# xiaoxubeii/kubernetes-schedule-simulator

Hardware: AMD Instinct MI355X
Metric: pods scheduled/sec + node-evals/sec at 100k nodes, 1/2/4/8 MI355X (higher is better)
Workload: dtype int64; 1 GPU; C3: 100000 nodes, 1000000-pod queue, default predicates + LeastRequested(1) + BalancedResourceAllocation(1); nodes=100000, global_batch=35715, mode=persistent, blocks=256, parallelism=single-gpu

## Files before the change

### kubernetes-schedule-simulator_amd/csrc/ksim_pfast.hip

```cpp
#include <algorithm>

#include "ksim_decide.h"
#include "ksim_f64.h"
#include "ksim_fast.h"
#include "ksim_phist.h"
#include "ksim_tree.h"
#include "ksim_wave.h"
#include "ksim_xchg.h"

using namespace kf64;

namespace {

#ifndef KSIM_PF_BS
#define KSIM_PF_BS 512
#endif
constexpr int BS = KSIM_PF_BS;
constexpr int NW = BS / 64;
constexpr int RW = NW - 1;
constexpr int RT = RW * 64;
constexpr int MAXB = 4;
constexpr int MAXG = 64 * MAXB;
constexpr int NSLOT = 4;
constexpr int FIXSTRIDE = 16;
constexpr int RING = 16;
constexpr int RING_FILL = 8;
constexpr uint64_t SPIN_LIMIT_TICKS = 200000000ull;
constexpr int ANSLOT = 8;

using ksimx::gu64;
__device__ __forceinline__ uint64_t* spec_at(uint64_t* gr, int slot, int b) {
  return gr + slot * MAXG + (b % MAXB) * 64 + b / MAXB;
}
__device__ __forceinline__ uint64_t* fix_at(uint64_t* gr, int slot) { return gr + NSLOT * MAXG + slot * FIXSTRIDE; }
#ifndef KSIM_NREP
#define KSIM_NREP 8
#endif
constexpr int NREP = KSIM_NREP;

constexpr int REP_STRIDE = 2112;
static_assert(NSLOT * MAXG + NSLOT * FIXSTRIDE <= REP_STRIDE, "replica overlap");

constexpr double EXACT_LIM = 281474976710656.0;
__device__ __forceinline__ uint32_t gtag(uint64_t v) { return (uint32_t)(v >> 56); }
__device__ __forceinline__ bool gstop(uint64_t v) { return (v >> 55) & 1; }
__device__ __forceinline__ int32_t gfit(uint64_t v) { return (int32_t)((v >> 42) & 0x1FFF); }
__device__ __forceinline__ int32_t gcnt(uint64_t v) { return (int32_t)((v >> 29) & 0x1FFF); }
__device__ __forceinline__ int32_t gscore(uint64_t v) { return ((int32_t)((uint32_t)v << 3)) >> 3; }
__device__ __forceinline__ uint64_t gpack(uint64_t tag, int32_t f, int32_t n, int32_t m) {
  return (tag << 56) | ((uint64_t)(uint32_t)f << 42) | ((uint64_t)(uint32_t)n << 29) | ((uint64_t)(uint32_t)m & 0x1FFFFFFFull);
}

__device__ __forceinline__ void lds_barrier() {
  __builtin_amdgcn_fence(__ATOMIC_RELEASE, "workgroup", "local");
  __builtin_amdgcn_s_barrier();
  __builtin_amdgcn_fence(__ATOMIC_ACQUIRE, "workgroup", "local");
}

#ifdef KSIM_PROBE
#define PROBE(k) do { if (KSIM_PROBE == (k)) __builtin_amdgcn_s_sleep(8); } while (0)
#else
#define PROBE(k) do { } while (0)
#endif

#ifdef KSIM_STAMPS
#define STAMP(k)                                       \
  do {                                                 \
    const uint64_t t_ = __builtin_amdgcn_s_memtime(); \
    st_acc[k] += t_ - t_prev;                         \
    t_prev = t_;                                      \
  } while (0)
#define OSTAMP(k)                                                          \
  do {                                                                     \
    const uint64_t t_ = __builtin_amdgcn_s_memtime();                     \
    if (lane == 0) atomicAdd((unsigned long long*)&a.dbg[k], t_ - o_prev); \
    o_prev = t_;                                                           \
  } while (0)
#else
#define STAMP(k) \
  do {           \
  } while (0)
#define OSTAMP(k) \
  do {            \
  } while (0)
#endif

}

struct PfArgs {
  int64_t n, chunk, first, end;
  const int64_t* alloc_cpu;
  const int64_t* alloc_mem;
  const int32_t* allowed_pods;
  const uint32_t* flags;
  int64_t* req_cpu;
  int64_t* req_mem;
  int64_t* nz_cpu;
  int64_t* nz_mem;
  int32_t* pod_count;
  const ksim_pod* pods;
  uint64_t* counter;
  int64_t* cursor;
  int32_t* out_node;
  int32_t* out_reasons;
  int32_t* err;
  uint64_t* dbg;
  uint64_t* granules;
  uint32_t preds;
  int32_t no_prio, collect;
  int32_t wl, wm, wb;
  int32_t rank, world;
  int64_t node_base;
  uint32_t xtag_base;
  uint64_t* xchg;
  uint64_t* peers[KSIM_MAX_RANKS];
  uint64_t start_ticks;
  double* mirror;
  const int32_t* tcls;
  const KsimTreeClass* tclass;
  int32_t ncls;
};

namespace {

struct FRows {
  double *ac, *am, *rc, *rm, *zc, *zm, *yc, *ym;
  int32_t *allowed, *count;
  uint32_t* fl;
  int32_t* ev;
  int32_t* ev2;
  uint32_t* rm2;
  uint32_t* rma;
  int16_t* cache;
  uint16_t* hist;
};

constexpr int LDS_ROW_BYTES = 8 * 8 + 8 * 4;
constexpr int LDS_ROW_BYTES_STREAM = 7 * 4;

extern __shared__ __attribute__((aligned(16))) char kf_smem[];

template <bool STREAM>
__device__ __forceinline__ FRows carve(int rows, const PfArgs& a, int64_t lo) {
  FRows r;
  if (STREAM) {
    double* m = a.mirror + lo;
    const int64_t n = a.n;
    r.ac = m; r.am = m + n; r.rc = m + 2 * n; r.rm = m + 3 * n;
    r.zc = m + 4 * n; r.zm = m + 5 * n; r.yc = nullptr; r.ym = nullptr;
    r.allowed = const_cast<int32_t*>(a.allowed_pods) + lo;
    r.count = a.pod_count + lo;
    r.fl = const_cast<uint32_t*>(a.flags) + lo;
    int32_t* q = reinterpret_cast<int32_t*>(kf_smem);
    r.ev = q;
    r.ev2 = q + 2 * rows;
    r.rm2 = reinterpret_cast<uint32_t*>(q + 3 * rows);
    r.rma = r.rm2 + 2 * rows;
    r.cache = nullptr;
    r.hist = nullptr;
    return r;
  }
  double* d = reinterpret_cast<double*>(kf_smem);
  r.ac = d; r.am = d + rows; r.rc = d + 2 * rows; r.rm = d + 3 * rows;
  r.zc = d + 4 * rows; r.zm = d + 5 * rows; r.yc = d + 6 * rows; r.ym = d + 7 * rows;
  int32_t* q = reinterpret_cast<int32_t*>(d + 8 * rows);
  r.allowed = q; r.count = q + rows;
  r.fl = reinterpret_cast<uint32_t*>(q + 2 * rows);
  r.ev = q + 3 * rows;
  r.ev2 = q + 5 * rows;
  r.rm2 = reinterpret_cast<uint32_t*>(q + 6 * rows);
  r.cache = reinterpret_cast<int16_t*>(q + 8 * rows);
  r.hist = reinterpret_cast<uint16_t*>(reinterpret_cast<char*>(r.cache) + (((size_t)a.ncls * rows * 2 + 15) & ~(size_t)15));
  return r;
}

typedef __attribute__((address_space(1))) const uint64_t cgu64;
typedef __attribute__((address_space(1))) const int32_t cgi32;
__device__ __forceinline__ double ld_l2(const double* p) {
  return __builtin_bit_cast(double, __hip_atomic_load((cgu64*)p, __ATOMIC_RELAXED, __HIP_MEMORY_SCOPE_AGENT));
}
__device__ __forceinline__ int32_t ld_l2(const int32_t* p) {
  return __hip_atomic_load((cgi32*)p, __ATOMIC_RELAXED, __HIP_MEMORY_SCOPE_AGENT);
}
__device__ __forceinline__ FRow load_frow_l2(const FRows& R, int32_t j) {
  FRow r;
  r.ac = ld_l2(R.ac + j); r.am = ld_l2(R.am + j); r.rc = ld_l2(R.rc + j); r.rm = ld_l2(R.rm + j);
  r.zc = ld_l2(R.zc + j); r.zm = ld_l2(R.zm + j);
  r.yc = r.ac != 0.0 ? 1.0 / r.ac : 0.0;
  r.ym = r.am != 0.0 ? 1.0 / r.am : 0.0;
  r.allowed = ld_l2(R.allowed + j); r.count = ld_l2(R.count + j);
  r.fl = (uint32_t)ld_l2(reinterpret_cast<const int32_t*>(R.fl) + j);
  return r;
}

template <bool STREAM>
__device__ __forceinline__ FRow load_frow(const FRows& R, int32_t j) {
  FRow r;
  r.ac = R.ac[j]; r.am = R.am[j]; r.rc = R.rc[j]; r.rm = R.rm[j]; r.zc = R.zc[j]; r.zm = R.zm[j];
  if (STREAM) {
    r.yc = r.ac != 0.0 ? 1.0 / r.ac : 0.0;
    r.ym = r.am != 0.0 ? 1.0 / r.am : 0.0;
  } else {
    r.yc = R.yc[j]; r.ym = R.ym[j];
  }
  r.allowed = R.allowed[j]; r.count = R.count[j]; r.fl = R.fl[j];
  return r;
}

struct Top2 {
  int32_t f, m1, c1, m2, c2;
};

}

template <int NPT, bool STREAM, bool CACHE, bool HIST = false>
__global__ __launch_bounds__(BS) void ksim_pfast_kernel(PfArgs a) {
  static_assert(!(STREAM && CACHE), "the cached form keeps the rows in LDS");
  static_assert(!HIST || CACHE, "the histograms count the cached evaluations");
  __shared__ int32_t s_wst[HIST ? 1 : 2][HIST ? 1 : RW][5];
  __shared__ uint64_t s_bm[2][NPT][RW];
  __shared__ int32_t s_wg[2][5];
  __shared__ int32_t s_fix[2][2];
  __shared__ int32_t s_hist[KSIM_NREASONS];
  __shared__ int32_t s_mode[2], s_own[2];
  __shared__ int32_t s_arr;
  __shared__ int32_t s_prow[2];
  __shared__ double s_pdel[2][4];
  __shared__ double s_pval[4];
  __shared__ int32_t s_pcnt;
  __shared__ __attribute__((aligned(16))) ksim_pod s_pod[RING];
  __shared__ int32_t s_pcls[CACHE ? RING : 1];
  __shared__ KsimTreeClass s_tcl[CACHE ? KSIM_TREE_MAX_CLASSES : 1];
#ifdef KSIM_STAMPS
  uint64_t st_acc[16] = {};
#endif

  const int tid = threadIdx.x, lane = tid & 63, wv = tid >> 6;
  const int rt = tid - 64;
  const int G = gridDim.x;
  const int me = blockIdx.x;
  const int64_t chunk = a.chunk;
  const int64_t lo = (int64_t)me * chunk;
  const int64_t hi = (lo + chunk < a.n) ? lo + chunk : a.n;
  const int32_t nrows = (int32_t)(hi - lo);
  const FRows R = carve<STREAM>((int)chunk, a, lo);
  const uint32_t preds = a.preds;
  const bool no_prio = a.no_prio != 0;
  const EvCfg EC = make_evcfg(preds, no_prio, a.wl, a.wm, a.wb);
  int32_t* const top_list = reinterpret_cast<int32_t*>(R.rm2 + chunk);
  uint64_t* const granules = a.granules;
  constexpr int NR = STREAM ? 1 : NREP;
  uint64_t* const my_rep = NR == 1 ? granules : granules + (me % NR) * REP_STRIDE;

  for (int32_t j = tid; j < (STREAM ? 0 : nrows); j += BS) {
    const int64_t i = lo + j;
    const double ac = (double)a.alloc_cpu[i], am = (double)a.alloc_mem[i];
    R.ac[j] = ac; R.am[j] = am;
    R.yc[j] = ac != 0.0 ? 1.0 / ac : 0.0;
    R.ym[j] = am != 0.0 ? 1.0 / am : 0.0;
    R.rc[j] = (double)a.req_cpu[i]; R.rm[j] = (double)a.req_mem[i];
    R.zc[j] = (double)a.nz_cpu[i]; R.zm[j] = (double)a.nz_mem[i];
    R.allowed[j] = a.allowed_pods[i]; R.count[j] = a.pod_count[i]; R.fl[j] = a.flags[i];
  }
  auto ring_load = [&](int64_t p0, uint4& v, int32_t& cl) {
    const int64_t p = p0 + lane / 8;
    if (p < a.end) v = reinterpret_cast<const uint4*>(&a.pods[p])[lane % 8];
    if (CACHE && lane < RING_FILL && p0 + lane < a.end) cl = a.tcls[p0 + lane];
  };
  auto ring_store = [&](int64_t p0, const uint4& v, int32_t cl) {
    const int64_t p = p0 + lane / 8;
    if (p < a.end) reinterpret_cast<uint4*>(&s_pod[p % RING])[lane % 8] = v;
    if (CACHE && lane < RING_FILL && p0 + lane < a.end) s_pcls[(p0 + lane) % RING] = cl;
  };
  uint4 ring_next = make_uint4(0, 0, 0, 0);
  int32_t ring_next_cl = 0;
  if (wv == 1) {
    uint4 v;
    int32_t cl = 0;
    ring_load(a.first, v, cl);
    ring_load(a.first + RING_FILL, ring_next, ring_next_cl);
    ring_store(a.first, v, cl);
  }
  if (CACHE)
    for (int k = tid; k < a.ncls; k += BS) s_tcl[k] = a.tclass[k];
  if (tid == 0) { s_fix[a.first & 1][0] = -1; s_arr = 0; s_prow[0] = s_prow[1] = -1; }
  uint64_t counter = *a.counter;
  __syncthreads();
  auto cls_fpod = [&](int k) -> FPod {
    const KsimTreeClass& t = s_tcl[k];
    return FPod{t.rq_c, t.rq_m, t.nz_c, t.nz_m, 0.0, 0.0, t.anyreq, t.be};
  };
  if (CACHE) {
    const int tot = a.ncls * nrows;
    uint32_t* const hw = reinterpret_cast<uint32_t*>(R.hist);
    if (HIST) {
      for (int i = tid; i < a.ncls * (KSIM_PHIST_BUCKETS / 2); i += BS) hw[i] = 0;
      __syncthreads();
    }
    for (int idx = tid; idx < tot; idx += BS) {
      const int k = idx / nrows, j = idx - k * nrows;
      uint32_t rm;
      const int32_t ev = feval(EC, cls_fpod(k), load_frow<false>(R, j), rm);
      R.cache[k * chunk + j] = (int16_t)ev;
      if (HIST && ev >= 0) atomicAdd(&hw[k * (KSIM_PHIST_BUCKETS / 2) + khist::word(ev)], khist::unit(ev));
    }
    __syncthreads();
  }

  auto ptag = [&](int64_t p) -> uint64_t { return (uint64_t)((p - a.first + 1) & 0xFF); };
  auto wave_stats = [&](const int32_t (&e)[NPT], int buf, int w) {
    int32_t v = -1, nf = 0;
#pragma unroll
    for (int k = 0; k < NPT; ++k) {
      nf += __popcll(__ballot(e[k] >= 0));
      v = e[k] > v ? e[k] : v;
    }
    const int32_t m1 = ksimw::max_i32(v);
    int32_t v2 = -1;
#pragma unroll
    for (int k = 0; k < NPT; ++k) v2 = (e[k] < m1 && e[k] > v2) ? e[k] : v2;
    const int32_t m2 = ksimw::max_i32(v2);
    int32_t c1 = 0, c2 = 0;
#pragma unroll
    for (int k = 0; k < NPT; ++k) {
      const uint64_t bm = m1 < 0 ? 0ull : __ballot(e[k] == m1);
      c1 += __popcll(bm);
      c2 += m2 < 0 ? 0 : __popcll(__ballot(e[k] == m2));
      if (lane == 0) s_bm[buf][k][w - 1] = bm;
    }
    if (lane == 0) {
      s_wst[buf][w - 1][0] = nf; s_wst[buf][w - 1][1] = m1; s_wst[buf][w - 1][2] = c1;
      s_wst[buf][w - 1][3] = m2; s_wst[buf][w - 1][4] = c2;
    }
  };
  auto arrive_publish = [&](int64_t p, int buf) {
    __builtin_amdgcn_fence(__ATOMIC_RELEASE, "workgroup", "local");
    int32_t old = 0;
    if (lane == 0) old = atomicAdd(&s_arr, 1);
    old = __builtin_amdgcn_readfirstlane(old);
    if ((old + 1) % RW == 0) {
      __builtin_amdgcn_fence(__ATOMIC_ACQUIRE, "workgroup", "local");
      const bool in = lane < RW;
      const int w = in ? lane : 0;
      const int32_t f = in ? s_wst[buf][w][0] : 0;
      const int32_t a1 = s_wst[buf][w][1], n1 = in ? s_wst[buf][w][2] : 0;
      const int32_t a2 = s_wst[buf][w][3], n2 = in ? s_wst[buf][w][4] : 0;
      Top2 t;
      t.f = ksimw::sum_i32(f);
      t.m1 = ksimw::max_i32(n1 ? a1 : -1);
      t.c1 = ksimw::sum_i32((n1 && a1 == t.m1) ? n1 : 0);
      t.m2 = ksimw::max_i32(n1 && a1 < t.m1 ? a1 : (n2 ? a2 : -1));
      t.c2 = ksimw::sum_i32(((n1 && a1 == t.m2) ? n1 : 0) + ((n2 && a2 == t.m2) ? n2 : 0));
      if (t.m2 < 0) t.c2 = 0;
      if (lane == 0) {
        s_wg[buf][0] = t.f; s_wg[buf][1] = t.m1; s_wg[buf][2] = t.c1; s_wg[buf][3] = t.m2; s_wg[buf][4] = t.c2;
        if (NR == 1) ksimx::store_agent((gu64*)spec_at(granules, (int)(p % NSLOT), me), gpack(ptag(p), t.f, t.c1, t.m1));
      }
      if (NR > 1 && lane < NR)
        ksimx::store_agent((gu64*)spec_at(granules + lane * REP_STRIDE, (int)(p % NSLOT), me), gpack(ptag(p), t.f, t.c1, t.m1));
    }
  };
  auto hist_publish = [&](int64_t p, int buf) {
    const int cls = s_pcls[p % RING];
    const int32_t h = R.hist[cls * KSIM_PHIST_BUCKETS + lane];
    const int32_t M = khist::top(__ballot(h != 0));
    if (wv == 1) {
      const int32_t F = ksimw::sum_i32(h);
      const int32_t C = __builtin_amdgcn_readlane(h, M < 0 ? 0 : M);
      if (lane == 0) {
        s_wg[buf][0] = F; s_wg[buf][1] = M; s_wg[buf][2] = C;
        if (NR == 1) ksimx::store_agent((gu64*)spec_at(granules, (int)(p % NSLOT), me), gpack(ptag(p), F, C, M));
      }
      if (NR > 1 && lane < NR)
        ksimx::store_agent((gu64*)spec_at(granules + lane * REP_STRIDE, (int)(p % NSLOT), me), gpack(ptag(p), F, C, M));
    }
    const int16_t* c1 = R.cache + cls * chunk;
#pragma unroll
    for (int k = 0; k < NPT; ++k) {
      const int32_t j = k * RT + rt;
      const uint64_t bm = __ballot(M >= 0 && j < nrows && (int32_t)c1[j] == M);
      if (lane == 0) s_bm[buf][k][wv - 1] = bm;
    }
  };
  struct Segs {
    uint64_t m;
    int32_t cnt, base, total;
  };
  auto seg_prepare = [&](int buf) -> Segs {
    constexpr int S = NPT * RW;
    const int32_t M = s_wg[buf][1];
    Segs sg;
    sg.m = 0;
    if (lane < S) {
      const int k = NPT - 1 - lane / RW, w = RW - 1 - lane % RW;
      if constexpr (HIST) sg.m = M >= 0 ? s_bm[buf][k][w] : 0ull;
      else sg.m = (M >= 0 && s_wst[buf][w][1] == M) ? s_bm[buf][k][w] : 0ull;
    }
    sg.cnt = __popcll(sg.m);
    const int32_t incl = ksimw::prefix_incl_i32(sg.cnt);
    sg.base = incl - sg.cnt;
    sg.total = __builtin_amdgcn_readlane(incl, 63);
    return sg;
  };
  auto seg_select = [&](const Segs& sg, int32_t rank) -> int32_t {
    const uint64_t hs = __ballot(sg.cnt != 0 && rank >= sg.base && rank < sg.base + sg.cnt);
    if (rank >= sg.total || !hs) return -1;
    const int t = __builtin_ctzll(hs);
    const uint64_t ms = ((uint64_t)(uint32_t)__builtin_amdgcn_readlane((int32_t)(sg.m >> 32), t) << 32) |
                        (uint64_t)(uint32_t)__builtin_amdgcn_readlane((int32_t)sg.m, t);
    const int32_t r = rank - __builtin_amdgcn_readlane(sg.base, t);
    const uint64_t hb = __ballot(((ms >> lane) & 1ull) && __popcll(ms >> lane) - 1 == r);
    if (!hb) return -1;
    const int k = NPT - 1 - t / RW, w = RW - 1 - t % RW;
    return k * RT + w * 64 + __builtin_ctzll(hb);
  };

  auto build_top_list = [&](int buf) {
    constexpr int S = NPT * RW;
    const int32_t M = s_wg[buf][1];
    uint64_t m = 0;
    if (lane < S) {
      const int k = NPT - 1 - lane / RW, w = RW - 1 - lane % RW;
      m = (M >= 0 && s_wst[buf][w][1] == M) ? s_bm[buf][k][w] : 0ull;
    }
    const int32_t cnt = __popcll(m);
    const int32_t base = ksimw::prefix_incl_i32(cnt) - cnt;
    uint64_t live = __ballot(cnt != 0);
    while (live) {
      const int t = __builtin_ctzll(live);
      live &= live - 1;
      const uint64_t ms = ((uint64_t)(uint32_t)__builtin_amdgcn_readlane((int32_t)(m >> 32), t) << 32) |
                          (uint64_t)(uint32_t)__builtin_amdgcn_readlane((int32_t)m, t);
      const int32_t b0 = __builtin_amdgcn_readlane(base, t);
      const int k = NPT - 1 - t / RW, w = RW - 1 - t % RW;
      if ((ms >> lane) & 1ull) top_list[b0 + __popcll(ms >> lane) - 1] = k * RT + w * 64 + lane;
    }
  };

  uint32_t A_rm[STREAM ? 1 : NPT], B_rm[STREAM ? 1 : NPT];
  if (wv > 0) {
    const FPod P0 = load_fpod(s_pod[a.first % RING]);
    int32_t e[NPT];
    int32_t* ev = R.ev + (a.first & 1) * chunk;
#pragma unroll
    for (int k = 0; k < NPT; ++k) {
      const int32_t j = k * RT + rt;
      e[k] = -1;
      uint32_t& am = A_rm[STREAM ? 0 : k];
      am = 0;
      if (CACHE) {
        if (j < nrows) e[k] = R.cache[s_pcls[a.first % RING] * chunk + j];
      } else if (j < nrows) {
        e[k] = feval(EC, P0, load_frow<STREAM>(R, j), am);
        if (STREAM) R.rma[(a.first & 1) * chunk + j] = am;
        ev[j] = e[k];
      }
    }
    if constexpr (HIST) {
      hist_publish(a.first, (int)(a.first & 1));
    } else {
      wave_stats(e, (int)(a.first & 1), wv);
      arrive_publish(a.first, (int)(a.first & 1));
    }
  }
  int X = -1;
  int64_t stop_at = a.end;
  lds_barrier();
#ifdef KSIM_STAMPS
  uint64_t t_prev = __builtin_amdgcn_s_memtime();
  uint64_t tb_prev = t_prev, bw_busy = 0, bw_wait = 0;
#endif

  int64_t last = a.first;
  for (int64_t pod = a.first; pod < a.end; ++pod) {
    last = pod;
    const bool has_next = pod + 1 < a.end;
    const int pb = (int)(pod & 1);
    const int nb = (int)((pod + 1) & 1);
    int32_t jsel = -1;
    uint64_t stopbit = 0;
    FRow jrow;
    int32_t e_new = -1;
    uint32_t m_new = 0;
    int32_t hM_old = -1, hM_new = -1;
    int32_t hcls = 0, hrow = 0, hF0 = 0;
    int32_t he_old = -1;
    double hdel[4] = {0.0, 0.0, 0.0, 0.0};
#ifdef KSIM_STAMPS
    uint64_t o_prev = 0;
#endif

    if (wv == 0) {
      Segs sg{};
      if (STREAM) build_top_list(pb);
      else sg = seg_prepare(pb);
      if constexpr (HIST) {
        if (has_next) {
          hcls = s_pcls[(pod + 1) % RING];
          hrow = R.hist[hcls * KSIM_PHIST_BUCKETS + lane];
          hF0 = ksimw::sum_i32(hrow);
          hM_old = khist::top(__ballot(hrow != 0));
        }
        const ksim_pod& Pp = s_pod[pod % RING];
        hdel[0] = (double)Pp.add_cpu; hdel[1] = (double)Pp.add_mem; hdel[2] = (double)Pp.nz_cpu; hdel[3] = (double)Pp.nz_mem;
      }
      STAMP(1);
      const uint64_t tag = ptag(pod);
      const int slot = (int)(pod % NSLOT);
      uint64_t g[MAXB], fx = 0;
      bool ok = false;
      const uint64_t t0 = __builtin_amdgcn_s_memrealtime();
      for (;;) {
#pragma unroll
        for (int j = 0; j < MAXB; ++j) g[j] = ksimx::load_agent((gu64*)my_rep + slot * MAXG + j * 64 + lane);
        fx = ksimx::load_agent((gu64*)fix_at(my_rep, slot));
        bool mine = X < 0 || gtag(fx) == tag;
#pragma unroll
        for (int j = 0; j < MAXB; ++j) {
          const int b = lane * MAXB + j;
          mine &= (b >= G) || b == X || gtag(g[j]) == tag;
        }
        if (__all(mine)) {
          ok = true;
#pragma unroll
          for (int j = 0; j < MAXB; ++j) g[j] = (lane * MAXB + j == X) ? fx : g[j];
          break;
        }
        if (__builtin_amdgcn_s_memrealtime() - t0 > SPIN_LIMIT_TICKS) break;
        __builtin_amdgcn_s_sleep(1);
      }
      STAMP(2);
      PROBE(3);
      int32_t f = 0, lm = -1;
#pragma unroll
      for (int j = 0; j < MAXB; ++j) {
        g[j] = (lane * MAXB + j < G) ? g[j] : 0;
        f += gfit(g[j]);
        lm = (gcnt(g[j]) && gscore(g[j]) > lm) ? gscore(g[j]) : lm;
      }
      const int32_t Fl = ksimw::sum_i32(f);
      const int32_t Ml = ksimw::max_i32(lm);
      int32_t bm[MAXB], tot = 0;
#pragma unroll
      for (int j = 0; j < MAXB; ++j) {
        bm[j] = (gcnt(g[j]) && gscore(g[j]) == Ml) ? gcnt(g[j]) : 0;
        tot += bm[j];
      }
      const int32_t pre = ksimw::prefix_incl_i32(tot);
      const int32_t Cl = __builtin_amdgcn_readlane(pre, 63);
      int32_t F = Fl, M0 = Ml;
      uint32_t C = (uint32_t)Cl;
      int64_t above_r = 0;
      bool stop_any = ok && X >= 0 && gstop(fx);
      if (a.world > 1 && ok) {
        const uint64_t at = (uint64_t)(uint32_t)(a.xtag_base + (uint32_t)(pod - a.first) + 1u) << 32;
        const int aslot = (int)(pod % ANSLOT);
        if (me == 0 && lane < a.world) {
          uint64_t* dst = a.peers[lane] + ((int64_t)aslot * KSIM_MAX_RANKS + a.rank) * 4;
          ksimx::store_system(dst, at | (uint32_t)Fl);
          ksimx::store_system(dst + 1, at | (stop_any ? 0x80000000ull : 0ull) | (uint32_t)Cl);
          ksimx::store_system(dst + 2, at | (uint32_t)Ml);
        }
        const bool rl = lane < a.world;
        const uint64_t* src = a.xchg + ((int64_t)aslot * KSIM_MAX_RANKS + (rl ? lane : 0)) * 4;
        uint64_t w0 = 0, w1 = 0, w2 = 0;
        const uint64_t hi = 0xFFFFFFFF00000000ull;
        for (;;) {
          w0 = ksimx::load_system(src);
          w1 = ksimx::load_system(src + 1);
          w2 = ksimx::load_system(src + 2);
          if (__all(!rl || ((w0 & hi) == at && (w1 & hi) == at && (w2 & hi) == at))) break;
          const uint64_t lim = (pod == a.first) ? a.start_ticks : SPIN_LIMIT_TICKS;
          if (__builtin_amdgcn_s_memrealtime() - t0 > lim) { ok = false; break; }
          __builtin_amdgcn_s_sleep(1);
        }
        const int32_t Fr = rl ? (int32_t)(uint32_t)w0 : 0, Cr = rl ? (int32_t)((uint32_t)w1 & 0x7FFFFFFFu) : 0;
        const int32_t Mr = (rl && Cr) ? (int32_t)(uint32_t)w2 : -1;
        F = ksimw::sum_i32(Fr);
        M0 = ksimw::max_i32(Mr);
        const int32_t Cm = (Cr && Mr == M0) ? Cr : 0;
        const int32_t pr = ksimw::prefix_incl_i32(Cm);
        C = (uint32_t)__builtin_amdgcn_readlane(pr, 63);
        above_r = (int64_t)C - __builtin_amdgcn_readlane(pr, a.rank);
        stop_any = __any(rl && ((w1 >> 31) & 1));
      }
      const uint32_t Cs = C ? C : 1u;
      const int64_t ix = ksim_select_ix(counter, Cs);
      const int64_t ixl = ix - above_r;
      const int64_t above = (int64_t)Cl - pre;
      const bool hit = Ml == M0 && tot > 0 && ixl >= above && ixl < above + tot;
      int32_t found = -1;
      int64_t rr = ixl - above;
#pragma unroll
      for (int j = MAXB - 1; j >= 0; --j) {
        const bool here = found < 0 && rr < bm[j];
        found = here ? lane * MAXB + j : found;
        rr = (found < 0) ? rr - bm[j] : rr;
      }
      const uint64_t hb = __ballot(hit);
      const int src = __builtin_ffsll((long long)hb) - 1;
      const int blk = hb ? __builtin_amdgcn_readlane(found, src) : -1;
      const int rank = hb ? __builtin_amdgcn_readlane((int32_t)rr, src) : 0;
      int mode;
      if (!ok) mode = -1;
      else if (stop_any) mode = -2;
      else if (F == 0) mode = 0;
      else if (hb) mode = blk >= 0 ? 2 : -1;
      else mode = a.world > 1 ? 3 : -1;
      if (mode >= 2 && F > 1) counter += 1;
      if (lane == 0 && mode == -1) atomicOr(a.err, ok ? 2 : 4);
      STAMP(3);
#ifdef KSIM_STAMPS
      o_prev = __builtin_amdgcn_s_memtime();
#endif
      if (mode == 2 && blk == me) {
        jsel = STREAM ? (rank < s_wg[pb][2] ? top_list[rank] : -1) : seg_select(sg, rank);
        if (jsel < 0 || jsel >= nrows) {
          jsel = -1;
          mode = -1;
          if (lane == 0) atomicOr(a.err, 2);
        } else if (HIST) {
          const double s0 = R.rc[jsel] + hdel[0], s1 = R.rm[jsel] + hdel[1], s2 = R.zc[jsel] + hdel[2], s3 = R.zm[jsel] + hdel[3];
          if (has_next) he_old = (int32_t)R.cache[hcls * chunk + jsel];
          stopbit = ((s0 >= EXACT_LIM) | (s1 >= EXACT_LIM) | (s2 >= EXACT_LIM) | (s3 >= EXACT_LIM)) ? (1ull << 55) : 0ull;
        } else if (!STREAM) {
          const ksim_pod& Pp = s_pod[pod % RING];
          stopbit = (R.rc[jsel] + (double)Pp.add_cpu >= EXACT_LIM || R.rm[jsel] + (double)Pp.add_mem >= EXACT_LIM ||
                     R.zc[jsel] + (double)Pp.nz_cpu >= EXACT_LIM || R.zm[jsel] + (double)Pp.nz_mem >= EXACT_LIM)
                        ? (1ull << 55)
                        : 0ull;
        } else if (has_next) {
          jrow = load_frow_l2(R, jsel);
          if (jsel != s_prow[nb]) {
            const FRow r2 = plus(jrow, load_fpod(s_pod[pod % RING]));
            e_new = feval(EC, load_fpod(s_pod[(pod + 1) % RING]), r2, m_new);
            stopbit = (r2.rc >= EXACT_LIM || r2.rm >= EXACT_LIM || r2.zc >= EXACT_LIM || r2.zm >= EXACT_LIM) ? (1ull << 55) : 0ull;
          }
        }
        OSTAMP(22);
      }
      if ((mode == 0 || mode == 3) && me == 0 && lane == 0) a.out_node[pod] = mode == 0 ? -1 : -2;
      if (lane == 0) {
        s_mode[pb] = mode;
        s_own[pb] = jsel;
        if (STREAM) {
          s_prow[pb] = jsel;
          if (jsel >= 0) {
            const ksim_pod& Pp = s_pod[pod % RING];
            s_pdel[pb][0] = (double)Pp.add_cpu; s_pdel[pb][1] = (double)Pp.add_mem;
            s_pdel[pb][2] = (double)Pp.nz_cpu; s_pdel[pb][3] = (double)Pp.nz_mem;
          }
        }
      }
      X = mode == 2 ? blk : -1;
      STAMP(6);
    } else {
      const int32_t prow = STREAM ? s_prow[nb] : -1;
      auto apply_commit = [&](FRow& r, int32_t j) {
        r.rc += s_pdel[nb][0]; r.rm += s_pdel[nb][1]; r.zc += s_pdel[nb][2]; r.zm += s_pdel[nb][3]; r.count += 1;
        R.rc[j] = r.rc; R.rm[j] = r.rm; R.zc[j] = r.zc; R.zm[j] = r.zm; R.count[j] = r.count;
        s_pval[0] = r.rc; s_pval[1] = r.rm; s_pval[2] = r.zc; s_pval[3] = r.zm; s_pcnt = r.count;
      };
      if (STREAM && !has_next && prow >= 0) {
#pragma unroll
        for (int k = 0; k < NPT; ++k) {
          const int32_t j = k * RT + rt;
          if (j == prow) {
            FRow r = load_frow<STREAM>(R, j);
            apply_commit(r, j);
          }
        }
      }
      if (has_next) {
      const bool refill = wv == 1 && ((pod - a.first) % RING_FILL) == 0;
      if (refill) ring_store(pod + RING_FILL, ring_next, ring_next_cl);
      uint4 rv;
      int32_t rcl = 0;
      if (refill) ring_load(pod + 2 * RING_FILL, rv, rcl);
#ifdef KSIM_STAMPS
      const uint64_t te0 = __builtin_amdgcn_s_memtime();
#endif
      PROBE(4);
      const FPod P = load_fpod(s_pod[pod % RING]);
      const FPod Q = load_fpod(s_pod[(pod + 1) % RING]);
#ifdef KSIM_STAMPS
      uint64_t tw = __builtin_amdgcn_s_memtime();
      if (tid == 64) st_acc[8] += tw - te0;
#define WSTAMP(k) do { const uint64_t t_ = __builtin_amdgcn_s_memtime(); if (tid == 64) st_acc[k] += t_ - tw; tw = t_; } while (0)
#else
#define WSTAMP(k) do { } while (0)
#endif
      int32_t e[NPT];
      FRow rk[STREAM ? 1 : NPT];
      int32_t* evn = R.ev + nb * chunk;
      if (CACHE) {
        if constexpr (HIST) {
          WSTAMP(9);
          hist_publish(pod + 1, nb);
          WSTAMP(10);
        } else {
          const int16_t* c1 = R.cache + s_pcls[(pod + 1) % RING] * chunk;
#pragma unroll
          for (int k = 0; k < NPT; ++k) {
            const int32_t j = k * RT + rt;
            e[k] = j < nrows ? (int32_t)c1[j] : -1;
          }
          WSTAMP(9);
          wave_stats(e, nb, wv);
          WSTAMP(10);
          arrive_publish(pod + 1, nb);
        }
        const int32_t M0 = s_wg[pb][1];
        const int16_t* c0 = R.cache + s_pcls[pod % RING] * chunk;
#pragma unroll
        for (int k = 0; k < NPT; ++k) {
          const int32_t j = k * RT + rt;
          if (M0 >= 0 && j < nrows && (int32_t)c0[j] == M0) {
            uint32_t m2;
            R.ev2[j] = feval(EC, Q, plus(load_frow<false>(R, j), P), m2);
            R.rm2[j] = m2;
          }
        }
      } else {
#pragma unroll
      for (int k = 0; k < NPT; ++k) {
        const int32_t j = k * RT + rt;
        e[k] = -1;
        uint32_t& bm = B_rm[STREAM ? 0 : k];
        bm = 0;
        if (j < nrows) {
          FRow r = load_frow<STREAM>(R, j);
          if (STREAM && j == prow) apply_commit(r, j);
          e[k] = feval(EC, Q, r, bm);
          evn[j] = e[k];
          if (STREAM) {
            R.rma[nb * chunk + j] = bm;
          } else {
            rk[STREAM ? 0 : k] = r;
          }
        }
      }
      WSTAMP(9);
      wave_stats(e, nb, wv);
      WSTAMP(10);
      PROBE(1);
      arrive_publish(pod + 1, nb);
      if (!STREAM) {
#pragma unroll
        for (int k = 0; k < NPT; ++k) {
          const int32_t j = k * RT + rt;
          if (j < nrows) {
            uint32_t m2;
            R.ev2[j] = feval(EC, Q, plus(rk[STREAM ? 0 : k], P), m2);
            R.rm2[j] = m2;
          }
        }
      }
      }
      WSTAMP(11);
#ifdef KSIM_STAMPS
      if (tid == 64) st_acc[5] += __builtin_amdgcn_s_memtime() - te0;
#endif
      if (refill) { ring_next = rv; ring_next_cl = rcl; }
      }
      if (STREAM && prow >= 0 && wv == 1 + (prow % RT) / 64) asm volatile("s_waitcnt vmcnt(0)" ::: "memory");
    }
#ifdef KSIM_STAMPS
    const uint64_t tb0 = __builtin_amdgcn_s_memtime();
#endif
    lds_barrier();
#ifdef KSIM_STAMPS
    {
      const uint64_t tb1 = __builtin_amdgcn_s_memtime();
      bw_busy += tb0 - tb_prev;
      bw_wait += tb1 - tb0;
      tb_prev = tb1;
    }
#endif
    STAMP(7);
    const int mode = s_mode[pb];
    if (mode < 0) {
      if (mode == -2) stop_at = pod;
      break;
    }
    const int32_t own = s_own[pb];

    if (own >= 0) {
      if (wv == 0) {
        OSTAMP(17);
        if (has_next) {
          if (STREAM && jsel == s_prow[nb]) {
            FRow r = jrow;
            r.rc = s_pval[0]; r.rm = s_pval[1]; r.zc = s_pval[2]; r.zm = s_pval[3]; r.count = s_pcnt;
            const FRow r2 = plus(r, load_fpod(s_pod[pod % RING]));
            e_new = feval(EC, load_fpod(s_pod[(pod + 1) % RING]), r2, m_new);
            stopbit = (r2.rc >= EXACT_LIM || r2.rm >= EXACT_LIM || r2.zc >= EXACT_LIM || r2.zm >= EXACT_LIM) ? (1ull << 55) : 0ull;
          }
          if (!STREAM) { e_new = R.ev2[jsel]; m_new = R.rm2[jsel]; }
          int32_t e_old, f0, m1 = -1, c1 = 0, m2 = -1, c2 = 0;
          if constexpr (HIST) {
            e_old = he_old;
            f0 = hF0;
          } else {
            e_old = CACHE ? (int32_t)R.cache[s_pcls[(pod + 1) % RING] * chunk + jsel] : R.ev[nb * chunk + jsel];
            f0 = s_wg[nb][0]; m1 = s_wg[nb][1]; c1 = s_wg[nb][2]; m2 = s_wg[nb][3]; c2 = s_wg[nb][4];
          }
          const bool rem = e_old >= 0, add = e_new >= 0;
          const int32_t Ff = f0 - (rem ? 1 : 0) + (add ? 1 : 0);
          int32_t M, Cn;
          if constexpr (HIST) {
            const int32_t h = khist::adjusted(hrow, lane, e_old, e_new);
            M = khist::top(__ballot(h != 0));
            Cn = __builtin_amdgcn_readlane(h, M < 0 ? 0 : M);
            hM_new = M;
          } else {
            const int32_t c1a = c1 - ((rem && e_old == m1) ? 1 : 0);
            const int32_t mb = c1a ? m1 : (c2 ? m2 : -1), cb = c1a ? c1a : c2;
            const bool up = add && (cb == 0 || e_new > mb), eq = add && !up && e_new == mb;
            M = up ? e_new : mb;
            Cn = up ? 1 : cb + (eq ? 1 : 0);
          }
          PROBE(2);
          if (NR > 1 && lane < NR)
            ksimx::store_agent((gu64*)fix_at(granules + lane * REP_STRIDE, (int)((pod + 1) % NSLOT)),
                          gpack(ptag(pod + 1), Ff, Cn, Cn ? M : -1) | stopbit);
          if (lane == 0) {
            if (NR == 1)
              ksimx::store_agent((gu64*)fix_at(granules, (int)((pod + 1) % NSLOT)), gpack(ptag(pod + 1), Ff, Cn, Cn ? M : -1) | stopbit);
            s_wg[nb][0] = Ff; s_wg[nb][1] = Cn ? M : -1; s_wg[nb][2] = Cn;
          }
        }
        OSTAMP(18);
        if (CACHE) {
          const FRow r2 = plus(load_frow<false>(R, jsel), load_fpod(s_pod[pod % RING]));
          if (lane < a.ncls) {
            uint32_t rm;
            const int32_t en = feval(EC, cls_fpod(lane), r2, rm);
            if constexpr (HIST) khist::move(R.hist + lane * KSIM_PHIST_BUCKETS, (int32_t)R.cache[lane * chunk + jsel], en);
            R.cache[lane * chunk + jsel] = (int16_t)en;
          }
        }
        if (lane == 0) {
          if (!STREAM) {
            const ksim_pod& Pp = s_pod[pod % RING];
            R.rc[jsel] += (double)Pp.add_cpu; R.rm[jsel] += (double)Pp.add_mem;
            R.zc[jsel] += (double)Pp.nz_cpu; R.zm[jsel] += (double)Pp.nz_mem;
            R.count[jsel] += 1;
          }
          if (stopbit) atomicOr(a.err, 8);
          a.out_node[pod] = (int32_t)(a.node_base + lo + jsel);
          if (has_next) {
            R.ev[nb * chunk + jsel] = e_new;
            s_fix[nb][0] = jsel;
            s_fix[nb][1] = (int32_t)m_new;
          } else {
            s_fix[nb][0] = -1;
          }
        }
      }
      lds_barrier();
      if (HIST && wv == 0 && has_next) {
        if (hM_new == hM_old) {
          if (lane == 0 && hM_new >= 0) {
            uint64_t& m = s_bm[nb][jsel / RT][(jsel % RT) / 64];
            const uint64_t bit = 1ull << (jsel & 63);
            m = e_new == hM_new ? (m | bit) : (m & ~bit);
          }
        } else {
          const int16_t* c1 = R.cache + s_pcls[(pod + 1) % RING] * chunk;
          for (int sgi = 0; sgi < NPT * RW; ++sgi) {
            const int32_t j = sgi * 64 + lane;
            const uint64_t bm = __ballot(hM_new >= 0 && j < nrows && (int32_t)c1[j] == hM_new);
            if (lane == 0) s_bm[nb][sgi / RW][sgi % RW] = bm;
          }
        }
        OSTAMP(19);
#ifdef KSIM_STAMPS
        if (lane == 0) atomicAdd((unsigned long long*)&a.dbg[21], 1ull);
#endif
      }
      if (!HIST && wv == 0 && has_next) {
        const int w = 1 + (jsel % RT) / 64;
        int32_t e[NPT];
#pragma unroll
        for (int k = 0; k < NPT; ++k) {
          const int32_t j = k * RT + (w - 1) * 64 + lane;
          e[k] = j < nrows ? (CACHE ? (int32_t)R.cache[s_pcls[(pod + 1) % RING] * chunk + j] : R.ev[nb * chunk + j]) : -1;
        }
        wave_stats(e, nb, w);
        OSTAMP(19);
#ifdef KSIM_STAMPS
        if (lane == 0) atomicAdd((unsigned long long*)&a.dbg[21], 1ull);
#endif
      }
    } else if (wv == 0 && lane == 0) {
      s_fix[nb][0] = -1;
    }

    if (mode == 0 && a.collect && a.out_reasons) {
      if (tid < KSIM_NREASONS) s_hist[tid] = 0;
      lds_barrier();
      if (wv > 0) {
        const int32_t fr = s_fix[pb][0];
        const uint32_t fmk = (uint32_t)s_fix[pb][1];
#pragma unroll
        for (int k = 0; k < NPT; ++k) {
          const int32_t j = k * RT + rt;
          uint32_t rm = (j == fr) ? fmk : !STREAM ? A_rm[STREAM ? 0 : k] : (j < nrows ? R.rma[pb * chunk + j] : 0u);
          if (CACHE) {
            rm = 0;
            if (j < nrows) (void)feval(EC, load_fpod(s_pod[pod % RING]), load_frow<false>(R, j), rm);
          }
          for (int r = 0; r < KSIM_NREASONS; ++r) {
            const int32_t n = __popcll(__ballot((rm >> r) & 1u));
            if (lane == 0 && n) atomicAdd(&s_hist[r], n);
          }
        }
      }
      lds_barrier();
      if (tid < KSIM_NREASONS && s_hist[tid]) atomicAdd(&a.out_reasons[pod * KSIM_NREASONS + tid], s_hist[tid]);
    }
    STAMP(4);
    if (wv > 0) {
#pragma unroll
      for (int k = 0; k < (STREAM ? 0 : NPT); ++k) A_rm[k] = B_rm[k];
    }
  }

  __syncthreads();
  if (STREAM) {
    if (tid == 0) {
      const int32_t pr = s_prow[last & 1];
      if (pr >= 0) {
        const double* d = s_pdel[last & 1];
        R.rc[pr] += d[0]; R.rm[pr] += d[1]; R.zc[pr] += d[2]; R.zm[pr] += d[3]; R.count[pr] += 1;
        if (R.rc[pr] >= EXACT_LIM || R.rm[pr] >= EXACT_LIM || R.zc[pr] >= EXACT_LIM || R.zm[pr] >= EXACT_LIM)
          atomicOr(a.err, 8);
      }
    }
    __syncthreads();
  }
  for (int32_t j = tid; j < nrows; j += BS) {
    const int64_t i = lo + j;
    a.req_cpu[i] = (int64_t)R.rc[j]; a.req_mem[i] = (int64_t)R.rm[j];
    a.nz_cpu[i] = (int64_t)R.zc[j]; a.nz_mem[i] = (int64_t)R.zm[j];
    a.pod_count[i] = R.count[j];
  }
  if (me == 0 && tid == 0) {
    *a.counter = counter;
    *a.cursor = stop_at;
  }
#ifdef KSIM_STAMPS
  if (me == 0 && lane == 0) {
    atomicAdd((unsigned long long*)&a.dbg[32 + wv], bw_busy);
    atomicAdd((unsigned long long*)&a.dbg[40 + wv], bw_wait);
  }
  if (me == 0 && tid == 0)
    for (int k = 0; k < 16; ++k) a.dbg[k] += (k == 5 || (k >= 8 && k <= 11)) ? 0 : st_acc[k];
  if (me == 0 && tid == 64)
    for (int k : {5, 8, 9, 10, 11}) a.dbg[k] += st_acc[k];
#endif
}

static constexpr int PF_LDS_BUDGET = 150 * 1024;

extern "C" int ksim_pfast_config(int64_t n, int max_grid, int stream, int* grid, int* lds_rows) {
  int dev = 0;
  hipDeviceProp_t p;
  if (hipGetDevice(&dev) != hipSuccess || hipGetDeviceProperties(&p, dev) != hipSuccess) return 0;
  int g = p.multiProcessorCount;
  if (max_grid > 0 && g > max_grid) g = max_grid;
  if (g <= 0 || n <= 0) return 0;
  if (g > MAXG) g = MAXG;
  if (n < (int64_t)g * 64) g = (int)((n + 63) / 64);
  if (g < 1) g = 1;
  const int64_t chunk = (n + g - 1) / g;
  if (stream) {
    if (chunk * LDS_ROW_BYTES_STREAM > PF_LDS_BUDGET || chunk > 9 * RT) return 0;
  } else if (chunk * LDS_ROW_BYTES > PF_LDS_BUDGET || chunk > 4 * RT) {
    return 0;
  }
  *grid = g;
  *lds_rows = (int)chunk;
  return 1;
}

extern "C" size_t ksim_pfast_granule_bytes(void) { return (size_t)NREP * REP_STRIDE * sizeof(uint64_t); }

extern "C" size_t ksim_shard_lx_offset(void) { return (size_t)ANSLOT * KSIM_MAX_RANKS * 4; }
extern "C" size_t ksim_shard_xchg_bytes(void) {
  return (ksim_shard_lx_offset() + (size_t)KSIM_LX_SLOTS * KSIM_MAX_RANKS * (KSIM_LX_REC + KSIM_PX_REC)) *
         sizeof(uint64_t);
}

__global__ __launch_bounds__(256) void ksim_pstream_prepare_kernel(const int64_t* __restrict__ ac, const int64_t* __restrict__ am,
                                                                    const int64_t* __restrict__ rc, const int64_t* __restrict__ rm,
                                                                    const int64_t* __restrict__ zc, const int64_t* __restrict__ zm,
                                                                    int64_t n, double* __restrict__ m) {
  for (int64_t i = (int64_t)blockIdx.x * blockDim.x + threadIdx.x; i < n; i += (int64_t)gridDim.x * blockDim.x) {
    const double dac = (double)ac[i], dam = (double)am[i];
    m[i] = dac;
    m[n + i] = dam;
    m[2 * n + i] = (double)rc[i];
    m[3 * n + i] = (double)rm[i];
    m[4 * n + i] = (double)zc[i];
// ... 94 lines not shown
```

### kubernetes-schedule-simulator_amd/csrc/ksim_phist.h

```cpp
#pragma once
#include <stdint.h>

#ifdef __HIPCC__
#include <hip/hip_runtime.h>
#define KSIM_PHIST_FN __host__ __device__ inline
#else
#define KSIM_PHIST_FN inline
#endif

#define KSIM_PHIST_BUCKETS 64

namespace khist {

KSIM_PHIST_FN int word(int s) { return s >> 1; }
KSIM_PHIST_FN uint32_t unit(int s) { return 1u << ((s & 1) * 16); }

KSIM_PHIST_FN void build(uint32_t* row, const int16_t* col, int n) {
  for (int s = 0; s < KSIM_PHIST_BUCKETS / 2; ++s) row[s] = 0;
  for (int j = 0; j < n; ++j)
    if (col[j] >= 0) row[word(col[j])] += unit(col[j]);
}

KSIM_PHIST_FN void move(uint16_t* row, int e_old, int e_new) {
  if (e_old == e_new) return;
  if (e_old >= 0) row[e_old] -= 1;
  if (e_new >= 0) row[e_new] += 1;
}

KSIM_PHIST_FN int32_t adjusted(int32_t h, int s, int e_old, int e_new) {
  return h - (s == e_old ? 1 : 0) + (s == e_new ? 1 : 0);
}

KSIM_PHIST_FN int top(uint64_t nonempty) { return nonempty ? 63 - __builtin_clzll(nonempty) : -1; }

KSIM_PHIST_FN void stats(const uint16_t* row, int e_old, int e_new, int32_t* F, int32_t* M, int32_t* C) {
  uint64_t ne = 0;
  int32_t f = 0;
  for (int s = 0; s < KSIM_PHIST_BUCKETS; ++s) {
    const int32_t h = adjusted(row[s], s, e_old, e_new);
    f += h;
    ne |= (uint64_t)(h != 0) << s;
  }
  const int m = top(ne);
  *F = f;
  *M = m;
  *C = m < 0 ? 0 : adjusted(row[m], m, e_old, e_new);
}

}
```

Baseline: 485,500 pods/s.

## Precompute per-candidate histogram fix granules speculatively in row waves

In the histogram path, the row waves now precompute, for every candidate row tied at the top score, the packed fix granule (fit count, max score, count, stop bit) that would result if that row were chosen. They store it in an LDS array and signal completion through per-wave done counters. Once the winner is known, the owning wave waits on the relevant done counter, reads the precomputed granule and publishes it immediately, instead of computing histogram adjustments on the critical path. The cost is extra speculative evaluations, an LDS spin-wait with a timeout error path, and reuse of the ev LDS region for the granule array.

```diff
diff --git a/kubernetes-schedule-simulator_amd/csrc/ksim_pfast.hip b/kubernetes-schedule-simulator_amd/csrc/ksim_pfast.hip
--- a/kubernetes-schedule-simulator_amd/csrc/ksim_pfast.hip
+++ b/kubernetes-schedule-simulator_amd/csrc/ksim_pfast.hip
@@ -133,6 +133,7 @@
   uint32_t* rma;
   int16_t* cache;
   uint16_t* hist;
+  uint64_t* fixg;
 };
 
 constexpr int LDS_ROW_BYTES = 8 * 8 + 8 * 4;
@@ -158,6 +159,7 @@
     r.rma = r.rm2 + 2 * rows;
     r.cache = nullptr;
     r.hist = nullptr;
+    r.fixg = nullptr;
     return r;
   }
   double* d = reinterpret_cast<double*>(kf_smem);
@@ -169,6 +171,7 @@
   r.ev = q + 3 * rows;
   r.ev2 = q + 5 * rows;
   r.rm2 = reinterpret_cast<uint32_t*>(q + 6 * rows);
+  r.fixg = reinterpret_cast<uint64_t*>(q + 3 * rows + (rows & 1));
   r.cache = reinterpret_cast<int16_t*>(q + 8 * rows);
   r.hist = reinterpret_cast<uint16_t*>(reinterpret_cast<char*>(r.cache) + (((size_t)a.ncls * rows * 2 + 15) & ~(size_t)15));
   return r;
@@ -224,6 +227,7 @@
   __shared__ int32_t s_hist[KSIM_NREASONS];
   __shared__ int32_t s_mode[2], s_own[2];
   __shared__ int32_t s_arr;
+  __shared__ uint32_t s_done[HIST ? RW : 1];
   __shared__ int32_t s_prow[2];
   __shared__ double s_pdel[2][4];
   __shared__ double s_pval[4];
@@ -283,6 +287,7 @@
   }
   if (CACHE)
     for (int k = tid; k < a.ncls; k += BS) s_tcl[k] = a.tclass[k];
+  if (HIST && tid < RW) s_done[tid] = 0;
   if (tid == 0) { s_fix[a.first & 1][0] = -1; s_arr = 0; s_prow[0] = s_prow[1] = -1; }
   uint64_t counter = *a.counter;
   __syncthreads();
@@ -360,13 +365,14 @@
         ksimx::store_agent((gu64*)spec_at(granules + lane * REP_STRIDE, (int)(p % NSLOT), me), gpack(ptag(p), t.f, t.c1, t.m1));
     }
   };
-  auto hist_publish = [&](int64_t p, int buf) {
+  auto hist_publish = [&](int64_t p, int buf) -> Top2 {
     const int cls = s_pcls[p % RING];
     const int32_t h = R.hist[cls * KSIM_PHIST_BUCKETS + lane];
-    const int32_t M = khist::top(__ballot(h != 0));
+    const uint64_t ne = __ballot(h != 0);
+    const int32_t M = khist::top(ne);
+    const int32_t F = ksimw::sum_i32(h);
+    const int32_t C = __builtin_amdgcn_readlane(h, M < 0 ? 0 : M);
     if (wv == 1) {
-      const int32_t F = ksimw::sum_i32(h);
-      const int32_t C = __builtin_amdgcn_readlane(h, M < 0 ? 0 : M);
       if (lane == 0) {
         s_wg[buf][0] = F; s_wg[buf][1] = M; s_wg[buf][2] = C;
         if (NR == 1) ksimx::store_agent((gu64*)spec_at(granules, (int)(p % NSLOT), me), gpack(ptag(p), F, C, M));
@@ -381,6 +387,8 @@
       const uint64_t bm = __ballot(M >= 0 && j < nrows && (int32_t)c1[j] == M);
       if (lane == 0) s_bm[buf][k][wv - 1] = bm;
     }
+    const int32_t M2 = khist::top(M < 0 ? 0ull : ne & ~(1ull << M));
+    return Top2{F, M, C, M2, M2 < 0 ? 0 : __builtin_amdgcn_readlane(h, M2 < 0 ? 0 : M2)};
   };
   struct Segs {
     uint64_t m;
@@ -457,7 +465,7 @@
       }
     }
     if constexpr (HIST) {
-      hist_publish(a.first, (int)(a.first & 1));
+      (void)hist_publish(a.first, (int)(a.first & 1));
     } else {
       wave_stats(e, (int)(a.first & 1), wv);
       arrive_publish(a.first, (int)(a.first & 1));
@@ -483,9 +491,7 @@
     int32_t e_new = -1;
     uint32_t m_new = 0;
     int32_t hM_old = -1, hM_new = -1;
-    int32_t hcls = 0, hrow = 0, hF0 = 0;
-    int32_t he_old = -1;
-    double hdel[4] = {0.0, 0.0, 0.0, 0.0};
+    uint64_t hfix = 0;
 #ifdef KSIM_STAMPS
     uint64_t o_prev = 0;
 #endif
@@ -494,16 +500,6 @@
       Segs sg{};
       if (STREAM) build_top_list(pb);
       else sg = seg_prepare(pb);
-      if constexpr (HIST) {
-        if (has_next) {
-          hcls = s_pcls[(pod + 1) % RING];
-          hrow = R.hist[hcls * KSIM_PHIST_BUCKETS + lane];
-          hF0 = ksimw::sum_i32(hrow);
-          hM_old = khist::top(__ballot(hrow != 0));
-        }
-        const ksim_pod& Pp = s_pod[pod % RING];
-        hdel[0] = (double)Pp.add_cpu; hdel[1] = (double)Pp.add_mem; hdel[2] = (double)Pp.nz_cpu; hdel[3] = (double)Pp.nz_mem;
-      }
       STAMP(1);
       const uint64_t tag = ptag(pod);
       const int slot = (int)(pod % NSLOT);
@@ -620,9 +616,35 @@
           mode = -1;
           if (lane == 0) atomicOr(a.err, 2);
         } else if (HIST) {
-          const double s0 = R.rc[jsel] + hdel[0], s1 = R.rm[jsel] + hdel[1], s2 = R.zc[jsel] + hdel[2], s3 = R.zm[jsel] + hdel[3];
-          if (has_next) he_old = (int32_t)R.cache[hcls * chunk + jsel];
-          stopbit = ((s0 >= EXACT_LIM) | (s1 >= EXACT_LIM) | (s2 >= EXACT_LIM) | (s3 >= EXACT_LIM)) ? (1ull << 55) : 0ull;
+          OSTAMP(22);
+          if (has_next) {
+            const uint32_t need = (uint32_t)(pod - a.first + 1);
+            auto short_of = [&]() -> bool {
+              const uint32_t d = __hip_atomic_load(&s_done[(jsel % RT) / 64], __ATOMIC_RELAXED, __HIP_MEMORY_SCOPE_WORKGROUP);
+              return (int32_t)((uint32_t)__builtin_amdgcn_readfirstlane((int32_t)d) - need) < 0;
+            };
+            bool done = true;
+            if (short_of()) {
+              OSTAMP(18);
+              const uint64_t tw0 = __builtin_amdgcn_s_memrealtime();
+              do {
+                if (__builtin_amdgcn_s_memrealtime() - tw0 > SPIN_LIMIT_TICKS) { done = false; break; }
+                __builtin_amdgcn_s_sleep(1);
+              } while (short_of());
+              OSTAMP(12);
+            }
+            __builtin_amdgcn_fence(__ATOMIC_ACQUIRE, "workgroup", "local");
+            if (!done) {
+              jsel = -1;
+              mode = -1;
+              if (lane == 0) atomicOr(a.err, 2);
+            } else {
+              hfix = R.fixg[jsel];
+              if (NR > 1 && lane < NR) ksimx::store_agent((gu64*)fix_at(granules + lane * REP_STRIDE, (int)((pod + 1) % NSLOT)), hfix);
+              if (NR == 1 && lane == 0) ksimx::store_agent((gu64*)fix_at(granules, (int)((pod + 1) % NSLOT)), hfix);
+            }
+          }
+          OSTAMP(18);
         } else if (!STREAM) {
           const ksim_pod& Pp = s_pod[pod % RING];
           stopbit = (R.rc[jsel] + (double)Pp.add_cpu >= EXACT_LIM || R.rm[jsel] + (double)Pp.add_mem >= EXACT_LIM ||
@@ -637,7 +659,7 @@
             stopbit = (r2.rc >= EXACT_LIM || r2.rm >= EXACT_LIM || r2.zc >= EXACT_LIM || r2.zm >= EXACT_LIM) ? (1ull << 55) : 0ull;
           }
         }
-        OSTAMP(22);
+        if (!HIST) OSTAMP(22);
       }
       if ((mode == 0 || mode == 3) && me == 0 && lane == 0) a.out_node[pod] = mode == 0 ? -1 : -2;
       if (lane == 0) {
@@ -694,9 +716,10 @@
       FRow rk[STREAM ? 1 : NPT];
       int32_t* evn = R.ev + nb * chunk;
       if (CACHE) {
+        Top2 ht{};
         if constexpr (HIST) {
           WSTAMP(9);
-          hist_publish(pod + 1, nb);
+          ht = hist_publish(pod + 1, nb);
           WSTAMP(10);
         } else {
           const int16_t* c1 = R.cache + s_pcls[(pod + 1) % RING] * chunk;
@@ -717,9 +740,22 @@
           const int32_t j = k * RT + rt;
           if (M0 >= 0 && j < nrows && (int32_t)c0[j] == M0) {
             uint32_t m2;
-            R.ev2[j] = feval(EC, Q, plus(load_frow<false>(R, j), P), m2);
-            R.rm2[j] = m2;
-          }
+            const FRow r2 = plus(load_frow<false>(R, j), P);
+            const int32_t en = feval(EC, Q, r2, m2);
+            if constexpr (HIST) {
+              int32_t Ff, Mf, Cf;
+              khist::fix(ht.f, ht.m1, ht.c1, ht.m2, ht.c2, (int32_t)R.cache[s_pcls[(pod + 1) % RING] * chunk + j], en, &Ff, &Mf, &Cf);
+              const bool stop = (r2.rc >= EXACT_LIM) | (r2.rm >= EXACT_LIM) | (r2.zc >= EXACT_LIM) | (r2.zm >= EXACT_LIM);
+              R.fixg[j] = gpack(ptag(pod + 1), Ff, Cf, Mf) | (stop ? (1ull << 55) : 0ull);
+            } else {
+              R.ev2[j] = en;
+              R.rm2[j] = m2;
+            }
+          }
+        }
+        if constexpr (HIST) {
+          __builtin_amdgcn_fence(__ATOMIC_RELEASE, "workgroup", "local");
+          if (lane == 0) __hip_atomic_store(&s_done[wv - 1], (uint32_t)(pod - a.first + 1), __ATOMIC_RELAXED, __HIP_MEMORY_SCOPE_WORKGROUP);
         }
       } else {
 #pragma unroll
@@ -788,7 +824,13 @@
     if (own >= 0) {
       if (wv == 0) {
         OSTAMP(17);
-        if (has_next) {
+        if constexpr (HIST) {
+          if (has_next) {
+            hM_old = s_wg[nb][1];
+            hM_new = gscore(hfix);
+            if (lane == 0) { s_wg[nb][0] = gfit(hfix); s_wg[nb][1] = hM_new; s_wg[nb][2] = gcnt(hfix); }
+          }
+        } else if (has_next) {
           if (STREAM && jsel == s_prow[nb]) {
             FRow r = jrow;
             r.rc = s_pval[0]; r.rm = s_pval[1]; r.zc = s_pval[2]; r.zm = s_pval[3]; r.count = s_pcnt;
@@ -797,29 +839,15 @@
             stopbit = (r2.rc >= EXACT_LIM || r2.rm >= EXACT_LIM || r2.zc >= EXACT_LIM || r2.zm >= EXACT_LIM) ? (1ull << 55) : 0ull;
           }
           if (!STREAM) { e_new = R.ev2[jsel]; m_new = R.rm2[jsel]; }
-          int32_t e_old, f0, m1 = -1, c1 = 0, m2 = -1, c2 = 0;
-          if constexpr (HIST) {
-            e_old = he_old;
-            f0 = hF0;
-          } else {
-            e_old = CACHE ? (int32_t)R.cache[s_pcls[(pod + 1) % RING] * chunk + jsel] : R.ev[nb * chunk + jsel];
-            f0 = s_wg[nb][0]; m1 = s_wg[nb][1]; c1 = s_wg[nb][2]; m2 = s_wg[nb][3]; c2 = s_wg[nb][4];
-          }
+          const int32_t e_old = CACHE ? (int32_t)R.cache[s_pcls[(pod + 1) % RING] * chunk + jsel] : R.ev[nb * chunk + jsel];
+          const int32_t f0 = s_wg[nb][0], m1 = s_wg[nb][1], c1 = s_wg[nb][2], m2 = s_wg[nb][3], c2 = s_wg[nb][4];
           const bool rem = e_old >= 0, add = e_new >= 0;
           const int32_t Ff = f0 - (rem ? 1 : 0) + (add ? 1 : 0);
-          int32_t M, Cn;
-          if constexpr (HIST) {
-            const int32_t h = khist::adjusted(hrow, lane, e_old, e_new);
-            M = khist::top(__ballot(h != 0));
-            Cn = __builtin_amdgcn_readlane(h, M < 0 ? 0 : M);
-            hM_new = M;
-          } else {
-            const int32_t c1a = c1 - ((rem && e_old == m1) ? 1 : 0);
-            const int32_t mb = c1a ? m1 : (c2 ? m2 : -1), cb = c1a ? c1a : c2;
-            const bool up = add && (cb == 0 || e_new > mb), eq = add && !up && e_new == mb;
-            M = up ? e_new : mb;
-            Cn = up ? 1 : cb + (eq ? 1 : 0);
-          }
+          const int32_t c1a = c1 - ((rem && e_old == m1) ? 1 : 0);
+          const int32_t mb = c1a ? m1 : (c2 ? m2 : -1), cb = c1a ? c1a : c2;
+          const bool up = add && (cb == 0 || e_new > mb), eq = add && !up && e_new == mb;
+          const int32_t M = up ? e_new : mb;
+          const int32_t Cn = up ? 1 : cb + (eq ? 1 : 0);
           PROBE(2);
           if (NR > 1 && lane < NR)
             ksimx::store_agent((gu64*)fix_at(granules + lane * REP_STRIDE, (int)((pod + 1) % NSLOT)),
@@ -830,15 +858,18 @@
             s_wg[nb][0] = Ff; s_wg[nb][1] = Cn ? M : -1; s_wg[nb][2] = Cn;
           }
         }
-        OSTAMP(18);
+        if (!HIST) OSTAMP(18);
         if (CACHE) {
           const FRow r2 = plus(load_frow<false>(R, jsel), load_fpod(s_pod[pod % RING]));
+          int32_t en = -1;
           if (lane < a.ncls) {
             uint32_t rm;
-            const int32_t en = feval(EC, cls_fpod(lane), r2, rm);
+            en = feval(EC, cls_fpod(lane), r2, rm);
             if constexpr (HIST) khist::move(R.hist + lane * KSIM_PHIST_BUCKETS, (int32_t)R.cache[lane * chunk + jsel], en);
             R.cache[lane * chunk + jsel] = (int16_t)en;
           }
+          if (HIST && has_next) e_new = __builtin_amdgcn_readlane(en, __builtin_amdgcn_readfirstlane(s_pcls[(pod + 1) % RING]));
+          if (HIST && (r2.rc >= EXACT_LIM || r2.rm >= EXACT_LIM || r2.zc >= EXACT_LIM || r2.zm >= EXACT_LIM)) stopbit = 1ull << 55;
         }
         if (lane == 0) {
           if (!STREAM) {
@@ -850,7 +881,7 @@
           if (stopbit) atomicOr(a.err, 8);
           a.out_node[pod] = (int32_t)(a.node_base + lo + jsel);
           if (has_next) {
-            R.ev[nb * chunk + jsel] = e_new;
+            if (!HIST) R.ev[nb * chunk + jsel] = e_new;
             s_fix[nb][0] = jsel;
             s_fix[nb][1] = (int32_t)m_new;
           } else {
diff --git a/kubernetes-schedule-simulator_amd/csrc/ksim_phist.h b/kubernetes-schedule-simulator_amd/csrc/ksim_phist.h
--- a/kubernetes-schedule-simulator_amd/csrc/ksim_phist.h
+++ b/kubernetes-schedule-simulator_amd/csrc/ksim_phist.h
@@ -47,4 +47,23 @@
   *C = m < 0 ? 0 : adjusted(row[m], m, e_old, e_new);
 }
 
+#ifndef KSIM_PHIST_TAKEN
+#define KSIM_PHIST_TAKEN(k) ((void)0)
+#endif
+
+KSIM_PHIST_FN void fix(int32_t F0, int M1, int32_t C1, int M2, int32_t C2, int e_old, int e_new, int32_t* F,
+                       int32_t* M, int32_t* C) {
+  const bool rem = e_old >= 0, add = e_new >= 0;
+  const int32_t c1a = C1 - ((rem && e_old == M1) ? 1 : 0);
+  const int mb = c1a ? M1 : (C2 ? M2 : -1);
+  const int32_t cb = c1a ? c1a : C2;
+  const bool up = add && (cb == 0 || e_new > mb), eq = add && !up && e_new == mb;
+  KSIM_PHIST_TAKEN(c1a != C1 ? 0 : 1);
+  KSIM_PHIST_TAKEN(c1a ? 2 : C2 ? 3 : 4);
+  KSIM_PHIST_TAKEN(!add ? 5 : up ? (cb == 0 ? 6 : 7) : eq ? 8 : 9);
+  *F = F0 - (rem ? 1 : 0) + (add ? 1 : 0);
+  *M = up ? e_new : mb;
+  *C = up ? 1 : cb + (eq ? 1 : 0);
 }
+
+}
```

After: 561,600 pods/s (median of 6 runs). 1.16x the previous value.
